# larskaislaniemi/PyLamp

Measured on AMD Instinct MI355X. Metric: stokes_heat_mic_cell_updates_per_s, higher is better.
Workload: dtype f64

## Files before the change

### pylamp_amd/csrc/pl_solver.hip

```cpp
#include "pl_internal.h"
#include <chrono>
#include <cmath>
#include <functional>
#include <limits>

#define TB(tab, k) (tab)[(k) + PL_TOFF]

void pl_launch_heat_rhs(pl_ctx* ctx, const PlHeatOp& op, const double* Told, const double* H, double* rhs);

template <typename T>
struct PlVvOpT {
    PlGeom g;
    const T* etas; const T* etan;
    const T *rdz, *rDz, *rdx, *rDx;
    int slave_x;
    int slave_z0, slave_zL;
    T s0, sL;
    const T* szz; const T* szx;
};
typedef PlVvOpT<double> PlVvOp;
typedef PlVvOpT<float> PlVvOpF;

enum { VV_ZERO = 0, VV_INT = 1, VV_SLAVE = 2 };

// ... 2317 lines not shown
}

template <int NS, int TS>
__global__ __launch_bounds__(mgt_nt(mgt_post_nn(NS, TS))) void k_mg_post(MgTileArgs a) {
    constexpr int H = NS, HC = H + 1, CR = TS + 2 * HC, NN = CR * CR, ECR = TS / 2 + H + 6, ENN = ECR * ECR, NPT = mgt_npt(NN), NT = mgt_nt(NN);
    __shared__ double V[2][2][NN];
    __shared__ double EC[2][ENN];
    __shared__ double TAB[4][CR + 4];
    double* const ES = V[0][0]; double* const EN = V[0][1];
    const PlGeom& g = a.op.g; const PlGeom& gc = a.opc.g;
    const int tid = threadIdx.x;
    const int ty = blockIdx.x / a.tiles_x, tx = blockIdx.x % a.tiles_x;
    const int ti0 = g.gi0 + ty * TS, tj0 = g.gj0 + tx * TS;
    const int ci0 = ti0 - HC, cj0 = tj0 - HC;
    MgtTab t; t.es = ES; t.en = EN; t.rdz = TAB[0]; t.rDz = TAB[1]; t.rdx = TAB[2]; t.rDx = TAB[3];
    mgt_load_table(TAB[0], a.op.rdz, ci0 - 1, CR + 3, g.nz); mgt_load_table(TAB[1], a.op.rDz, ci0 - 1, CR + 3, g.nz);
    mgt_load_table(TAB[2], a.op.rdx, cj0 - 1, CR + 3, g.nx); mgt_load_table(TAB[3], a.op.rDx, cj0 - 1, CR + 3, g.nx);
    const long long P = g.plane;
    const int eI0 = ((ti0 - H) >> 1) - 2, eJ0 = ((tj0 - H) >> 1) - 2;
    MgtC kz[NPT], kx[NPT];
    int depth[NPT];
#pragma unroll
    for (int q = 0; q < NPT; q++) {
        const int idx = tid + q * NT;
        const bool have = idx < NN;
        const int ra = have ? idx / CR : 0, rb = have ? idx % CR : 0, i = ci0 + ra, j = cj0 + rb;
        depth[q] = have ? min(min(ra, CR - 1 - ra), min(rb, CR - 1 - rb)) : -1;
        kz[q] = mgt_classify<true>(a.op, CR, CR, ci0, cj0, ra, rb);
        kx[q] = mgt_classify<false>(a.op, CR, CR, ci0, cj0, ra, rb);
        const bool inmem = i - g.gi0 >= -PL_RING && i - g.gi0 < g.lnz + PL_RING && j - g.gj0 >= -PL_RING && j - g.gj0 < g.lnx + PL_RING;
        const long long c = pl_idx(g, i - g.gi0, j - g.gj0);
        if (kz[q].on) kz[q].f = a.f[c + kz[q].d];
        if (kx[q].on) kx[q].f = a.f[c + (long long)kx[q].d * g.pitch + P];
        if (have) {
            ES[idx] = inmem ? a.op.etas[c] : 0.0; EN[idx] = inmem ? a.op.etan[c] : 0.0;
            V[1][0][idx] = inmem ? a.v[c] : 0.0; V[1][1][idx] = inmem ? a.v[c + P] : 0.0;
        }
    }
    for (int idx = tid; idx < ENN; idx += NT) {
        const int I = eI0 + idx / ECR, J = eJ0 + idx % ECR;
        const bool inmem = I - gc.gi0 >= -PL_RING && I - gc.gi0 < gc.lnz + PL_RING && J - gc.gj0 >= -PL_RING && J - gc.gj0 < gc.lnx + PL_RING;
        const long long cc = pl_idx(gc, I - gc.gi0, J - gc.gj0);
        EC[0][idx] = inmem ? a.ec[cc] : 0.0; EC[1][idx] = inmem ? a.ec[cc + gc.plane] : 0.0;
    }
    __syncthreads();
#pragma unroll
    for (int q = 0; q < NPT; q++) { mgt_coefficients<true>(kz[q], t, CR); mgt_coefficients<false>(kx[q], t, CR); }
    __syncthreads();
    auto ecz = [&](int I, int J) { return EC[0][(I - eI0) * ECR + (J - eJ0)]; };
    auto ecx = [&](int I, int J) { return EC[1][(I - eI0) * ECR + (J - eJ0)]; };
#pragma unroll
    for (int q = 0; q < NPT; q++) {
        const int idx = tid + q * NT;
        if (depth[q] >= HC - H) {
            const int ra = idx / CR, rb = idx % CR, i = ci0 + ra, j = cj0 + rb;
            int d; double s;
            double oz = 0.0, ox = 0.0;
            if (mgt_cls_z(a.op, i, j, d, s) != VV_ZERO) {
                const int jm = j + d;
                const int I0 = i >> 1, I1 = (i + 1) >> 1;
                int Jn = jm >> 1, Jo = (jm & 1) ? Jn + 1 : Jn - 1;
                Jn = min(max(Jn, 0), gc.nx - 2); Jo = min(max(Jo, 0), gc.nx - 2);
                const double pa = 0.5 * (ecz(I0, Jn) + ecz(I1, Jn)), pb = 0.5 * (ecz(I0, Jo) + ecz(I1, Jo));
                oz = s * (V[1][0][idx + d] + (0.75 * pa + 0.25 * pb));
            }
            if (mgt_cls_x(a.op, i, j, d, s) != VV_ZERO) {
                const int im = i + d;
                const int J0 = j >> 1, J1 = (j + 1) >> 1;
                int In = im >> 1, Io = (im & 1) ? In + 1 : In - 1;
                In = min(max(In, 0), gc.nz - 2); Io = min(max(Io, 0), gc.nz - 2);
                const double pa = 0.5 * (ecx(In, J0) + ecx(In, J1)), pb = 0.5 * (ecx(Io, J0) + ecx(Io, J1));
                ox = s * (V[1][1][idx + d * CR] + (0.75 * pa + 0.25 * pb));
            }
            V[0][0][idx] = oz; V[0][1][idx] = ox;
        }
    }
    __syncthreads();
    int cur = 0;
    double pvz[NPT], pvx[NPT];
#pragma unroll
    for (int q = 0; q < NPT; q++) { pvz[q] = 0.0; pvx[q] = 0.0; }
#pragma unroll
    for (int k = 0; k < NS; k++) {
        const int h = H - 1 - k;
#pragma unroll
        for (int q = 0; q < NPT; q++) {
            const int idx = tid + q * NT;
            if (depth[q] >= HC - h) {
                double oz, ox;
                mgt_cheb(kz[q], kx[q], CR, V[cur][0], V[cur][1], pvz[q], pvx[q], k == 0 ? 0.0 : a.c1[k], a.c2[k], oz, ox);
                if (k == NS - 1) {
                    const int ra = idx / CR, rb = idx % CR, i = ci0 + ra, j = cj0 + rb;
                    if (i < g.nz && j < g.nx && i - g.gi0 < g.lnz && j - g.gj0 < g.lnx) {
                        const long long c = pl_idx(g, i - g.gi0, j - g.gj0); a.out[c] = oz * a.oscale; a.out[c + a.out_plane] = ox * a.oscale;
                    }
                } else { V[cur ^ 1][0][idx] = oz; V[cur ^ 1][1][idx] = ox; }
            }
        }
        if (k < NS - 1) { __syncthreads(); cur ^= 1; }
    }
#pragma unroll
    for (int q = 0; q < NPT; q++) {
        const int idx = tid + q * NT;
        if (depth[q] == HC - 1) {
            const int ra = idx / CR, rb = idx % CR, i = ci0 + ra, j = cj0 + rb;
            if (mgt_owns(ra, rb, HC, TS, i, j, g) && i - g.gi0 < g.lnz && j - g.gj0 < g.lnx) {
                const long long c = pl_idx(g, i - g.gi0, j - g.gj0); a.out[c] = 0.0; a.out[c + a.out_plane] = 0.0;
            }
        }
    }
}

#define MGT_TAIL_POOL 18600
struct TailLvl { int base, NR, CR, N; };
#define TL_V(D, buf, c) (pool + (D).base + (2 * (buf) + (c)) * (D).N)
#define TL_F(D, c) (pool + (D).base + (6 + (c)) * (D).N)
#define TL_ES(D) (pool + (D).base + 8 * (D).N)
#define TL_EN(D) (pool + (D).base + 9 * (D).N)
#define TL_TAB(D, k) (pool + (D).base + 10 * (D).N + ((k) < 2 ? (k) * ((D).NR + 3) : 2 * ((D).NR + 3) + ((k) - 2) * ((D).CR + 3)))
#define TL_FOR_NODES(g)                                                                                                     \
    for (int idx = threadIdx.x, nxm_ = (g).nx - 1, pw_ = (nxm_ & (nxm_ - 1)) == 0, sh_ = 31 - __clz(nxm_), i, j;            \
         idx < ((g).nz - 1) * nxm_ && (i = pw_ ? idx >> sh_ : idx / nxm_, j = idx - i * nxm_, true); idx += MGT_NT)
__device__ inline MgtTile mgt_tail_tile(double* pool, const TailLvl& D) {
    MgtTile T; T.ci0 = -1; T.cj0 = -1; T.CR = D.CR; T.NR = D.NR;
    T.t.es = TL_ES(D); T.t.en = TL_EN(D); T.t.rdz = TL_TAB(D, 0); T.t.rDz = TL_TAB(D, 1); T.t.rdx = TL_TAB(D, 2); T.t.rDx = TL_TAB(D, 3);
    return T;
}
__device__ inline void mgt_tail_smooth(double* pool, const TailLevel& L, const TailLvl& D, int& cur, int& prv, int& nxt, int nsweep, double ratio, bool zero_guess) {
    const double lmax = L.lmax, lmin = lmax / ratio;
    const double theta = 0.5 * (lmax + lmin), delta = 0.5 * (lmax - lmin), sigma = theta / delta;
    double rho_old = 1.0 / sigma;
    const MgtTile T = mgt_tail_tile(pool, D);
    for (int k = 0; k < nsweep; k++) {
        double c1, c2;
        if (k == 0) { c1 = 0.0; c2 = 1.0 / theta; }
        else { const double rho = 1.0 / (2.0 * sigma - rho_old); c1 = rho * rho_old; c2 = 2.0 * rho / delta; rho_old = rho; }
        double* const nz_ = TL_V(D, nxt, 0); double* const nx_ = TL_V(D, nxt, 1);
        const double* const cz = TL_V(D, cur, 0); const double* const cx = TL_V(D, cur, 1);
        const bool noprev = k == 1 && zero_guess;
        const double* const pz = noprev ? nullptr : TL_V(D, prv, 0); const double* const px = noprev ? nullptr : TL_V(D, prv, 1);
        TL_FOR_NODES(L.op.g) {
            const int ra = i + 1, rb = j + 1;
            if (k == 0 && zero_guess) T.first(L.op, TL_F(D, 0), TL_F(D, 1), nz_, nx_, c2, ra, rb);
            else {
                double oz, ox;
                T.cheb(L.op, cz, cx, pz, px, TL_F(D, 0), TL_F(D, 1), c1, c2, ra, rb, oz, ox);
                nz_[ra * D.CR + rb] = oz; nx_[ra * D.CR + rb] = ox;
            }
        }
        __syncthreads();
        const int o = prv; prv = cur; cur = nxt; nxt = o;
    }
}
__global__ __launch_bounds__(MGT_NT) void k_mg_tail_lds(TailArgs a) {
    __shared__ double pool[MGT_TAIL_POOL];
    __shared__ TailLvl lv[PL_TAIL_MAX_LEVELS];
    __shared__ int rot[PL_TAIL_MAX_LEVELS];
    const int tid = threadIdx.x;
    for (int k = tid; k < MGT_TAIL_POOL; k += MGT_NT) pool[k] = 0.0;
    if (tid == 0) {
        int q = 0;
        for (int l = 0; l < a.nlev; l++) {
            const PlGeom& g = a.L[l].op.g;
            TailLvl D; D.base = q; D.NR = g.nz + 2; D.CR = g.nx + 2; D.N = D.NR * D.CR;
            q += 10 * D.N + 2 * (D.NR + 3) + 2 * (D.CR + 3);
            lv[l] = D;
        }
    }
    __syncthreads();
    for (int l = 0; l < a.nlev; l++) {
        const TailLevel& L = a.L[l]; const PlGeom& g = L.op.g; const TailLvl D = lv[l];
        for (int idx = tid; idx < g.nz * g.nx; idx += MGT_NT) {
            const int i = idx / g.nx, j = idx - i * g.nx;
            const long long c = pl_idx(g, i - g.gi0, j - g.gj0);
            const int o = (i + 1) * D.CR + (j + 1);
            TL_ES(D)[o] = L.op.etas[c]; TL_EN(D)[o] = L.op.etan[c];
            if (l == 0) { TL_F(D, 0)[o] = L.f[c]; TL_F(D, 1)[o] = L.f[c + g.plane]; }
        }
        mgt_load_table(TL_TAB(D, 0), L.op.rdz, -2, D.NR + 3, g.nz); mgt_load_table(TL_TAB(D, 1), L.op.rDz, -2, D.NR + 3, g.nz);
        mgt_load_table(TL_TAB(D, 2), L.op.rdx, -2, D.CR + 3, g.nx); mgt_load_table(TL_TAB(D, 3), L.op.rDx, -2, D.CR + 3, g.nx);
    }
    __syncthreads();
    for (int l = 0; l < a.nlev; l++) {
        const TailLevel& L = a.L[l]; const PlGeom& g = L.op.g; const TailLvl D = lv[l];
        int cur = 0, prv = 1, nxt = 2;
        if (l == a.nlev - 1) {
            double ratio = 0.4 * g.nz * g.nx; if (ratio < 30.0) ratio = 30.0;
            mgt_tail_smooth(pool, L, D, cur, prv, nxt, a.coarse_sweeps, ratio, true);
            if (tid == 0) rot[l] = cur | (prv << 2) | (nxt << 4);
            break;
        }
        mgt_tail_smooth(pool, L, D, cur, prv, nxt, a.nu_pre, a.ratio, true);
        if (tid == 0) rot[l] = cur | (prv << 2) | (nxt << 4);
        const MgtTile T = mgt_tail_tile(pool, D);
        double* const rz = TL_V(D, nxt, 0); double* const rx = TL_V(D, nxt, 1);
        const double* const cz = TL_V(D, cur, 0); const double* const cx = TL_V(D, cur, 1);
        TL_FOR_NODES(g) {
            const int ra = i + 1, rb = j + 1, o = ra * D.CR + rb;
            int d; double s, Av, dg, vz = 0.0, vx = 0.0;
            if (mgt_cls_z(L.op, i, j, d, s) == VV_INT) { mgt_row_z<true>(T.t, D.CR, cz, cx, o, ra, rb, Av, dg); vz = TL_F(D, 0)[o] - Av; }
            if (mgt_cls_x(L.op, i, j, d, s) == VV_INT) { mgt_row_x<true>(T.t, D.CR, cz, cx, o, ra, rb, Av, dg); vx = TL_F(D, 1)[o] - Av; }
            rz[o] = vz; rx[o] = vx;
        }
        __syncthreads();
        const TailLevel& Cn = a.L[l + 1]; const TailLvl Dc = lv[l + 1];
        double* const fz = TL_F(Dc, 0); double* const fx = TL_F(Dc, 1);
        TL_FOR_NODES(Cn.op.g) {
            const int b0 = (2 * i + 1) * D.CR + (2 * j + 1);
            int d; double s, oz = 0.0, ox = 0.0;
            if (vv_cls_z(Cn.op, i, j, d, s) == VV_INT) {
                const double wz[3] = {0.25, 0.5, 0.25}, wx[4] = {0.125, 0.375, 0.375, 0.125};
#pragma unroll
                for (int u = 0; u < 3; u++)
#pragma unroll
                    for (int w = 0; w < 4; w++) oz += wz[u] * wx[w] * rz[b0 + (u - 1) * D.CR + (w - 1)];
            }
            if (vv_cls_x(Cn.op, i, j, d, s) == VV_INT) {
                const double wz[4] = {0.125, 0.375, 0.375, 0.125}, wx[3] = {0.25, 0.5, 0.25};
#pragma unroll
                for (int u = 0; u < 4; u++)
#pragma unroll
                    for (int w = 0; w < 3; w++) ox += wz[u] * wx[w] * rx[b0 + (u - 1) * D.CR + (w - 1)];
            }
            const int oc = (i + 1) * Dc.CR + (j + 1);
            fz[oc] = oz; fx[oc] = ox;
        }
        __syncthreads();
    }
    __syncthreads();
    for (int l = a.nlev - 2; l >= 0; l--) {
        const TailLevel& L = a.L[l]; const PlGeom& g = L.op.g; const TailLvl D = lv[l];
        const PlGeom& gc = a.L[l + 1].op.g; const TailLvl Dc = lv[l + 1];
        int cur = rot[l] & 3, prv = (rot[l] >> 2) & 3, nxt = (rot[l] >> 4) & 3;
        const int curc = rot[l + 1] & 3;
        const double* const ez = TL_V(Dc, curc, 0); const double* const ex = TL_V(Dc, curc, 1);
        const double* const cz = TL_V(D, cur, 0); const double* const cx = TL_V(D, cur, 1);
        double* const wz_ = TL_V(D, nxt, 0); double* const wx_ = TL_V(D, nxt, 1);
        TL_FOR_NODES(g) {
            const int o = (i + 1) * D.CR + (j + 1);
            int d; double s, oz = 0.0, ox = 0.0;
            if (mgt_cls_z(L.op, i, j, d, s) != VV_ZERO) {
                const int jm = j + d, I0 = i >> 1, I1 = (i + 1) >> 1;
                int Jn = jm >> 1, Jo = (jm & 1) ? Jn + 1 : Jn - 1;
                Jn = min(max(Jn, 0), gc.nx - 2); Jo = min(max(Jo, 0), gc.nx - 2);
                const double pa = 0.5 * (ez[(I0 + 1) * Dc.CR + Jn + 1] + ez[(I1 + 1) * Dc.CR + Jn + 1]);
                const double pb = 0.5 * (ez[(I0 + 1) * Dc.CR + Jo + 1] + ez[(I1 + 1) * Dc.CR + Jo + 1]);
                oz = s * (cz[o + d] + (0.75 * pa + 0.25 * pb));
            }
            if (mgt_cls_x(L.op, i, j, d, s) != VV_ZERO) {
                const int im = i + d, J0 = j >> 1, J1 = (j + 1) >> 1;
                int In = im >> 1, Io = (im & 1) ? In + 1 : In - 1;
                In = min(max(In, 0), gc.nz - 2); Io = min(max(Io, 0), gc.nz - 2);
                const double pa = 0.5 * (ex[(In + 1) * Dc.CR + J0 + 1] + ex[(In + 1) * Dc.CR + J1 + 1]);
                const double pb = 0.5 * (ex[(Io + 1) * Dc.CR + J0 + 1] + ex[(Io + 1) * Dc.CR + J1 + 1]);
                ox = s * (cx[o + d * D.CR] + (0.75 * pa + 0.25 * pb));
            }
            wz_[o] = oz; wx_[o] = ox;
        }
        __syncthreads();
        { const int o = cur; cur = nxt; nxt = o; }
        mgt_tail_smooth(pool, L, D, cur, prv, nxt, a.nu_post, a.ratio, false);
        if (tid == 0) rot[l] = cur | (prv << 2) | (nxt << 4);
        __syncthreads();
    }
    {
        const TailLevel& L = a.L[0]; const PlGeom& g = L.op.g; const TailLvl D = lv[0];
        const int cur = rot[0] & 3;
        const double* const cz = TL_V(D, cur, 0); const double* const cx = TL_V(D, cur, 1);
        for (int idx = tid; idx < g.nz * g.nx; idx += MGT_NT) {
            const int i = idx / g.nx, j = idx - i * g.nx, o = (i + 1) * D.CR + (j + 1);
            const long long c = pl_idx(g, i - g.gi0, j - g.gj0);
            L.v[0][c] = cz[o]; L.v[0][c + g.plane] = cx[o];
        }
    }
}
static bool mg_tail_lds_fits(const PlSolver* S, size_t l) {
    long long need = 0;
    for (size_t q = l; q < S->levels.size(); q++) {
        const PlGeom& g = S->levels[q]->gh.d;
        need += 10LL * (g.nz + 2) * (g.nx + 2) + 2LL * (g.nz + 5) + 2LL * (g.nx + 5);
    }
    return need <= MGT_TAIL_POOL;
}

static void cheb_coeffs(double lmax, double ratio, int n, double* c1, double* c2) {
    const double lmin = lmax / ratio, theta = 0.5 * (lmax + lmin), delta = 0.5 * (lmax - lmin), sigma = theta / delta;
    double rho_old = 1.0 / sigma;
    for (int k = 0; k < n; k++) {
        if (k == 0) { c1[k] = 0.0; c2[k] = 1.0 / theta; }
        else { const double rho = 1.0 / (2.0 * sigma - rho_old); c1[k] = rho * rho_old; c2[k] = 2.0 * rho / delta; rho_old = rho; }
    }
}
static bool mg_fused_level_ok(pl_ctx* ctx, const PlSolver* S, size_t l) {
    if (!S->fused || l + 1 >= S->levels.size() || S->any_line) return false;
    const MgLevel* L = S->levels[l];
    if (L->f32 || L->op.szz) return false;
    const PlGeom& g = L->gh.d;
    int npre_, npost_;
    level_nu(S, l, npre_, npost_);
    if (L->dist) {
        const bool dist_fused = !(getenv("PYLAMP_MG_FUSED_DIST") && atoi(getenv("PYLAMP_MG_FUSED_DIST")) == 0);
        const MgLevel* C = S->levels[l + 1];
        if (!dist_fused || l == 0 || npre_ + 2 > std::min(g.lnz, g.lnx) || npre_ + 3 > PL_RING) return false;
        if (C->dist && std::min(C->gh.d.lnz, C->gh.d.lnx) < 4) return false;
        if ((g.gi0 & 1) || (g.gj0 & 1)) return false;
    } else if (S->levels[l + 1]->dist) return false;
    if ((long long)g.lnz * g.lnx > S->fused_max_nodes) return false;
    if (S->use_tail && l > 0 && (long long)g.nz * g.nx <= S->tail_max_nodes && S->levels.size() - l <= PL_TAIL_MAX_LEVELS) return false;
    int npre, npost;
    level_nu(S, l, npre, npost);
    return npre >= 1 && npre <= 3 && npost >= 1 && npost <= 3;
}
static void vcycle_fused_level(pl_ctx* ctx, PlSolver* S, size_t l, const double* f, double** out, double* final_out, double final_scale,
                               const PlStokesOp* sop, const double* rs, double* z) {
    MgLevel* L = S->levels[l];
    MgLevel* C = S->levels[l + 1];
    const PlGeom& g = L->gh.d;
    int npre, npost;
    level_nu(S, l, npre, npost);
    MgTileArgs a{};
    a.op = L->op; a.opc = C->op;
    a.f = rs ? (const double*)L->f : f; a.fout = L->f; a.v = L->v[0]; a.fc = C->f;
    const int TS = (long long)g.lnz * g.lnx >= S->tile32_min_nodes ? 32 : MGT_TS;
    const int own_z = g.lnz - (g.gi0 + g.lnz == g.nz ? 1 : 0), own_x = g.lnx - (g.gj0 + g.lnx == g.nx ? 1 : 0);
    a.tiles_x = (own_x + TS - 1) / TS;
    const dim3 grid((unsigned)(a.tiles_x * ((own_z + TS - 1) / TS)));
    cheb_coeffs(L->lmax, S->cheb_ratio, npre, a.c1, a.c2);
    if (rs) { a.sop = *sop; a.rs = rs; a.z = z; }
#define MGT_PRE(NS, L0) do { if (TS == 32) hipLaunchKernelGGL((k_mg_pre<NS, L0, 32>), grid, dim3(mgt_nt(mgt_pre_nn(NS, 32))), 0, ctx->stream, a); \
                             else hipLaunchKernelGGL((k_mg_pre<NS, L0, MGT_TS>), grid, dim3(mgt_nt(mgt_pre_nn(NS, MGT_TS))), 0, ctx->stream, a); } while (0)
#define MGT_PRE_X(NS) do { if (TS == 32) hipLaunchKernelGGL((k_mg_pre<NS, false, 32, 1>), grid, dim3(mgt_nt(mgt_pre_nn(NS + 1, 32))), 0, ctx->stream, a); \
                           else hipLaunchKernelGGL((k_mg_pre<NS, false, MGT_TS, 1>), grid, dim3(mgt_nt(mgt_pre_nn(NS + 1, MGT_TS))), 0, ctx->stream, a); } while (0)
    if (L->dist) {
        (void)pl_halo(ctx, g, (double*)a.f, 2, g.plane, npre + 2);
        if (npre == 1) MGT_PRE_X(1); else if (npre == 2) MGT_PRE_X(2); else MGT_PRE_X(3);
        if (!C->dist) (void)pl_gather_blocks(ctx, C->gh.d, C->f, 2, C->gh.d.plane);
    }
    else if (rs) { if (npre == 1) MGT_PRE(1, true); else if (npre == 2) MGT_PRE(2, true); else MGT_PRE(3, true); }
    else { if (npre == 1) MGT_PRE(1, false); else if (npre == 2) MGT_PRE(2, false); else MGT_PRE(3, false); }
#undef MGT_PRE
#undef MGT_PRE_X
    double* ec = nullptr;
    bool wf = false;
    vcycle<double>(ctx, S, l + 1, C->f, &ec, &wf, nullptr, 1.0, 0, nullptr);
    if (L->dist && C->dist) (void)pl_halo(ctx, C->gh.d, ec, 2, C->gh.d.plane, 4);
    a.ec = ec; a.out = final_out ? final_out : L->v[2]; a.oscale = final_out ? final_scale : 1.0; a.out_plane = g.plane;
    cheb_coeffs(L->lmax, S->cheb_ratio, npost, a.c1, a.c2);
#define MGT_POST(NS) do { if (TS == 32) hipLaunchKernelGGL((k_mg_post<NS, 32>), grid, dim3(mgt_nt(mgt_post_nn(NS, 32))), 0, ctx->stream, a); \
                          else hipLaunchKernelGGL((k_mg_post<NS, MGT_TS>), grid, dim3(mgt_nt(mgt_post_nn(NS, MGT_TS))), 0, ctx->stream, a); } while (0)
    if (npost == 1) MGT_POST(1); else if (npost == 2) MGT_POST(2); else MGT_POST(3);
#undef MGT_POST
    *out = final_out ? nullptr : L->v[2];
}

template <typename T>
__global__ __launch_bounds__(256) void k_copy_vel(PlGeom g, const T* __restrict__ e, double* __restrict__ z, double oscale) {
    PL_NODE_PROLOGUE(g)
    (void)i; (void)j;
    z[c] = (double)e[c] * oscale; z[c + g.plane] = (double)e[c + g.plane] * oscale;
}

__global__ __launch_bounds__(256) void k_vv_close_frame(PlVvOp op, double* __restrict__ z) {
    const PlGeom& g = op.g;
    const int t = blockIdx.x * 256 + threadIdx.x;
    int i, j;
    if (t < 3 * g.lnx) { const int q = t / g.lnx; i = q == 0 ? 0 : g.nz - 3 + q; j = g.gj0 + t % g.lnx; }
    else if (t < 3 * g.lnx + 3 * g.lnz) { const int u = t - 3 * g.lnx, q = u / g.lnz; j = q == 0 ? 0 : g.nx - 3 + q; i = g.gi0 + u % g.lnz; }
    else return;
    const int li = i - g.gi0, lj = j - g.gj0;
    if (li < 0 || li >= g.lnz || lj < 0 || lj >= g.lnx) return;
    const long long c = pl_idx(g, li, lj), P = g.plane;
    int moff; double s;
    int cls = vv_cls_z(op, i, j, moff, s);
    if (cls == VV_ZERO) z[c] = 0.0; else if (cls == VV_SLAVE) z[c] = s * z[c + moff];
    cls = vv_cls_x(op, i, j, moff, s);
    if (cls == VV_ZERO) z[c + P] = 0.0; else if (cls == VV_SLAVE) z[c + P] = s * z[c + moff + P];
}

template <typename T>
static int stokes_precond_t(pl_ctx* ctx, PlSolver* S, const double* rs, double* z) {
    PlStokesOp op = ctx->sop;
    MgLevel* L0 = S->levels[0];
    MgLevel* L = L0;
    const PlGeom& g = ctx->sop.g;
    const bool f32 = std::is_same<T, float>::value;
    const double kappa = f32 ? S->kappa : 1.0, fscale = f32 ? S->kappa / S->sigma : 1.0, oscale = f32 ? 1.0 / S->kappa : 1.0;
    int e_last = 0, f_depth = 0;
    const bool deep = level_deep_plan(S, L0, 0, e_last, f_depth);
    ExtViewT<T> V = ext_view<T>(ctx, L0, deep ? f_depth : 0);
    if (L0->dist) {
        if (deep) PL_TRY(pl_halo(ctx, g, (double*)rs, 3, g.plane, f_depth + 1));
        else PL_TRY(pl_halo(ctx, g, (double*)rs + 2 * g.plane, 1, g.plane));
    }
    op.g = V.op.g; op.etas -= V.sh; op.etan -= V.sh; if (op.rho) op.rho -= V.sh;
    op.iKc /= S->schur_scale;
    if constexpr (std::is_same<T, double>::value) {
        if (mg_fused_level_ok(ctx, S, 0)) {
            double* e2 = nullptr;
            vcycle_fused_level(ctx, S, 0, nullptr, &e2, z, 1.0, &op, rs, z);
            PL_HIP(ctx, hipGetLastError());
            S->nprec++;
            return 0;
        }
    }
    int npre0, npost0;
    level_nu(S, 0, npre0, npost0);
    if constexpr (std::is_same<T, double>::value) {
        const double hmean = 0.5 * ((ctx->geom.zc.back() - ctx->geom.zc.front()) / (ctx->nz - 1) + (ctx->geom.xc.back() - ctx->geom.xc.front()) / (ctx->nx - 1));
        const double sig = ctx->sop.Kc / hmean, ik = 1.0 / S->kappa;
        const bool range_ok = std::isfinite(sig) && sig > 0.0 && ik * std::min(1.0, sig) > 1e-30 && ik * std::max(1.0, sig) < 1e22;
        if (S->l0_mixed && S->l0_mixed_now && !S->any_line && range_ok && !L0->dist && !L0->op.szz && g_vv_vec && (g.plane % 2) == 0 && S->levels.size() > 1 && npre0 == 1 && npost0 == 1 &&
            S->fuse_first && ctx->nranks == 1 && !S->levels[1]->dist && !S->levels[1]->f32) {
            MgLevel* C = S->levels[1];
            for (float** q : {&L0->ff, &L0->rf, &L0->vf[0]}) if (!*q) PL_TRY(fmalloc0(ctx, q, (size_t)2 * g.plane * sizeof(float)));
            float* ff = L0->ff; float* rf = L0->rf; float* v1f = L0->vf[0];
            double* vd = L0->v[0];
            PlVvOpT<float> cls{};
// ... 1165 lines not shown
```

Measured before the change: 186.2 million.

## Run coarsest multigrid tail levels on a single wavefront with register-resident stencils

Restructures the LDS multigrid tail kernel so levels small enough to fit in one wavefront (at most 64 nodes) are processed by the first 64 threads only, using wave barriers instead of block-wide __syncthreads. Levels that fit in one block use a per-thread node path whose stencil coefficients and RHS are classified once and kept in registers, rather than recomputed each sweep. Chebyshev coefficients for every level's pre- and post-smoothing sequence are precomputed into a shared table. This targets barrier and recomputation latency in the tiny coarse levels, at the cost of more registers and code complexity, plus reliance on wavefront-synchronous LDS ordering.

Measured after the change: 188.3 million (median of 6 runs). 1.01x the previous value.

```diff
diff --git a/pylamp_amd/csrc/pl_solver.hip b/pylamp_amd/csrc/pl_solver.hip
--- a/pylamp_amd/csrc/pl_solver.hip
+++ b/pylamp_amd/csrc/pl_solver.hip
@@ -2493,8 +2493,171 @@
         const int o = prv; prv = cur; cur = nxt; nxt = o;
     }
 }
+struct TailNode { MgtC kz, kx; int o; bool have; };
+__device__ inline TailNode mgt_tail_enter(double* pool, const TailLevel& L, const TailLvl& D) {
+    TailNode n;
+    const int nxm = L.op.g.nx - 1, idx = threadIdx.x;
+    n.have = idx < (L.op.g.nz - 1) * nxm;
+    const int i = n.have ? idx / nxm : 0, j = n.have ? idx - i * nxm : 0;
+    n.o = (i + 1) * D.CR + (j + 1);
+    n.kz = mgt_classify<true>(L.op, D.CR, D.NR, -1, -1, i + 1, j + 1);
+    n.kx = mgt_classify<false>(L.op, D.CR, D.NR, -1, -1, i + 1, j + 1);
+    if (!n.have) { n.kz.on = n.kz.interior = false; n.kx.on = n.kx.interior = false; }
+    const MgtTile T = mgt_tail_tile(pool, D);
+    mgt_coefficients<true>(n.kz, T.t, D.CR); mgt_coefficients<false>(n.kx, T.t, D.CR);
+    if (n.kz.on) n.kz.f = TL_F(D, 0)[n.kz.cm];
+    if (n.kx.on) n.kx.f = TL_F(D, 1)[n.kx.cm];
+    return n;
+}
+template <bool WAVE> __device__ inline void mgt_tail_sync() {
+    if (WAVE) { asm volatile("s_waitcnt lgkmcnt(0)" ::: "memory"); __builtin_amdgcn_wave_barrier(); }
+    else __syncthreads();
+}
+struct MgtChebSeq {
+    double theta, delta, sigma, rho_old;
+    __device__ inline void init(double lmax, double ratio) {
+        const double lmin = lmax / ratio;
+        theta = 0.5 * (lmax + lmin); delta = 0.5 * (lmax - lmin); sigma = theta / delta; rho_old = 1.0 / sigma;
+    }
+    __device__ inline void next(int k, double& c1, double& c2) {
+        if (k == 0) { c1 = 0.0; c2 = 1.0 / theta; }
+        else { const double rho = 1.0 / (2.0 * sigma - rho_old); c1 = rho * rho_old; c2 = 2.0 * rho / delta; rho_old = rho; }
+    }
+};
+#define MGT_TAIL_CHEB 16
+#define MGT_TAIL_SEQ (2 * PL_TAIL_MAX_LEVELS)
+__device__ inline void mgt_tail_sequence(const TailArgs& a, int s, int& n, double& ratio) {
+    const int l = s % PL_TAIL_MAX_LEVELS;
+    const bool up = s >= PL_TAIL_MAX_LEVELS, coarsest = l == a.nlev - 1;
+    n = 0; ratio = a.ratio;
+    if (l >= a.nlev || (up && coarsest)) return;
+    n = up ? a.nu_post : (coarsest ? a.coarse_sweeps : a.nu_pre);
+    if (coarsest) { const PlGeom& g = a.L[l].op.g; ratio = 0.4 * g.nz * g.nx; if (ratio < 30.0) ratio = 30.0; }
+}
+template <bool WAVE>
+__device__ inline void mgt_tail_smooth_rows(double* pool, const TailLvl& D, const TailNode& n, const double (*ch)[MGT_TAIL_CHEB], double lmax, double ratio,
+                                            int& cur, int& prv, int& nxt, int nsweep, bool zero_guess) {
+    const bool table = nsweep <= MGT_TAIL_CHEB;
+    MgtChebSeq seq; seq.theta = seq.delta = seq.sigma = seq.rho_old = 1.0;
+    if (!table) seq.init(lmax, ratio);
+    double pvz = 0.0, pvx = 0.0;
+    for (int k = 0; k < nsweep; k++) {
+        double c1, c2;
+        if (table) { c1 = ch[0][k]; c2 = ch[1][k]; } else seq.next(k, c1, c2);
+        if (n.have) {
+            double oz, ox;
+            if (k == 0 && zero_guess) {
+                oz = n.kz.on ? (-n.kz.s * c2 * n.kz.f) * n.kz.rdg : 0.0;
+                ox = n.kx.on ? (-n.kx.s * c2 * n.kx.f) * n.kx.rdg : 0.0;
+            } else mgt_cheb(n.kz, n.kx, D.CR, TL_V(D, cur, 0), TL_V(D, cur, 1), pvz, pvx, c1, c2, oz, ox);
+            TL_V(D, nxt, 0)[n.o] = oz; TL_V(D, nxt, 1)[n.o] = ox;
+        }
+        mgt_tail_sync<WAVE>();
+        const int o = prv; prv = cur; cur = nxt; nxt = o;
+    }
+}
+template <bool WAVE>
+__device__ inline void mgt_tail_down(double* pool, const TailArgs& a, const TailLvl* lv, int* rot, const double (*chb)[2][MGT_TAIL_CHEB], int l) {
+    const TailLevel& L = a.L[l]; const PlGeom& g = L.op.g; const TailLvl D = lv[l];
+    const bool coarsest = l == a.nlev - 1, rows = (g.nz - 1) * (g.nx - 1) <= MGT_NT;
+    int cur = 0, prv = 1, nxt = 2, nsweep;
+    double ratio;
+    mgt_tail_sequence(a, l, nsweep, ratio);
+    if (rows) {
+        const TailNode n = mgt_tail_enter(pool, L, D);
+        mgt_tail_smooth_rows<WAVE>(pool, D, n, chb[l], L.lmax, ratio, cur, prv, nxt, nsweep, true);
+        if (threadIdx.x == 0) rot[l] = cur | (prv << 2) | (nxt << 4);
+        if (coarsest) { mgt_tail_sync<WAVE>(); return; }
+        if (n.have) {
+            double v0, vz = 0.0, vx = 0.0;
+            if (n.kz.interior) vz = n.kz.f - mgt_av_z(n.kz, D.CR, TL_V(D, cur, 0), TL_V(D, cur, 1), v0);
+            if (n.kx.interior) vx = n.kx.f - mgt_av_x(n.kx, D.CR, TL_V(D, cur, 0), TL_V(D, cur, 1), v0);
+            TL_V(D, nxt, 0)[n.o] = vz; TL_V(D, nxt, 1)[n.o] = vx;
+        }
+    } else if constexpr (!WAVE) {
+        mgt_tail_smooth(pool, L, D, cur, prv, nxt, nsweep, ratio, true);
+        if (threadIdx.x == 0) rot[l] = cur | (prv << 2) | (nxt << 4);
+        if (coarsest) { mgt_tail_sync<WAVE>(); return; }
+        const MgtTile T = mgt_tail_tile(pool, D);
+        const double* const cz = TL_V(D, cur, 0); const double* const cx = TL_V(D, cur, 1);
+        TL_FOR_NODES(g) {
+            const int ra = i + 1, rb = j + 1, o = ra * D.CR + rb;
+            int d; double s, Av, dg, vz = 0.0, vx = 0.0;
+            if (mgt_cls_z(L.op, i, j, d, s) == VV_INT) { mgt_row_z<true>(T.t, D.CR, cz, cx, o, ra, rb, Av, dg); vz = TL_F(D, 0)[o] - Av; }
+            if (mgt_cls_x(L.op, i, j, d, s) == VV_INT) { mgt_row_x<true>(T.t, D.CR, cz, cx, o, ra, rb, Av, dg); vx = TL_F(D, 1)[o] - Av; }
+            TL_V(D, nxt, 0)[o] = vz; TL_V(D, nxt, 1)[o] = vx;
+        }
+    }
+    mgt_tail_sync<WAVE>();
+    const double* const qz = TL_V(D, nxt, 0); const double* const qx = TL_V(D, nxt, 1);
+    const TailLevel& Cn = a.L[l + 1]; const TailLvl Dc = lv[l + 1];
+    double* const fz = TL_F(Dc, 0); double* const fx = TL_F(Dc, 1);
+    TL_FOR_NODES(Cn.op.g) {
+        const int b0 = (2 * i + 1) * D.CR + (2 * j + 1);
+        int d; double s, oz = 0.0, ox = 0.0;
+        if (vv_cls_z(Cn.op, i, j, d, s) == VV_INT) {
+            const double wz[3] = {0.25, 0.5, 0.25}, wx[4] = {0.125, 0.375, 0.375, 0.125};
+#pragma unroll
+            for (int u = 0; u < 3; u++)
+#pragma unroll
+                for (int w = 0; w < 4; w++) oz += wz[u] * wx[w] * qz[b0 + (u - 1) * D.CR + (w - 1)];
+        }
+        if (vv_cls_x(Cn.op, i, j, d, s) == VV_INT) {
+            const double wz[4] = {0.125, 0.375, 0.375, 0.125}, wx[3] = {0.25, 0.5, 0.25};
+#pragma unroll
+            for (int u = 0; u < 4; u++)
+#pragma unroll
+                for (int w = 0; w < 3; w++) ox += wz[u] * wx[w] * qx[b0 + (u - 1) * D.CR + (w - 1)];
+        }
+        const int oc = (i + 1) * Dc.CR + (j + 1);
+        fz[oc] = oz; fx[oc] = ox;
+    }
+    mgt_tail_sync<WAVE>();
+}
+template <bool WAVE>
+__device__ inline void mgt_tail_up(double* pool, const TailArgs& a, const TailLvl* lv, int* rot, const double (*chb)[2][MGT_TAIL_CHEB], int l) {
+    const TailLevel& L = a.L[l]; const PlGeom& g = L.op.g; const TailLvl D = lv[l];
+    const PlGeom& gc = a.L[l + 1].op.g; const TailLvl Dc = lv[l + 1];
+    int cur = rot[l] & 3, prv = (rot[l] >> 2) & 3, nxt = (rot[l] >> 4) & 3;
+    const int curc = rot[l + 1] & 3;
+    const double* const ez = TL_V(Dc, curc, 0); const double* const ex = TL_V(Dc, curc, 1);
+    const double* const cz = TL_V(D, cur, 0); const double* const cx = TL_V(D, cur, 1);
+    double* const wz_ = TL_V(D, nxt, 0); double* const wx_ = TL_V(D, nxt, 1);
+    TL_FOR_NODES(g) {
+        const int o = (i + 1) * D.CR + (j + 1);
+        int d; double s, oz = 0.0, ox = 0.0;
+        if (mgt_cls_z(L.op, i, j, d, s) != VV_ZERO) {
+            const int jm = j + d, I0 = i >> 1, I1 = (i + 1) >> 1;
+            int Jn = jm >> 1, Jo = (jm & 1) ? Jn + 1 : Jn - 1;
+            Jn = min(max(Jn, 0), gc.nx - 2); Jo = min(max(Jo, 0), gc.nx - 2);
+            const double pa = 0.5 * (ez[(I0 + 1) * Dc.CR + Jn + 1] + ez[(I1 + 1) * Dc.CR + Jn + 1]);
+            const double pb = 0.5 * (ez[(I0 + 1) * Dc.CR + Jo + 1] + ez[(I1 + 1) * Dc.CR + Jo + 1]);
+            oz = s * (cz[o + d] + (0.75 * pa + 0.25 * pb));
+        }
+        if (mgt_cls_x(L.op, i, j, d, s) != VV_ZERO) {
+            const int im = i + d, J0 = j >> 1, J1 = (j + 1) >> 1;
+            int In = im >> 1, Io = (im & 1) ? In + 1 : In - 1;
+            In = min(max(In, 0), gc.nz - 2); Io = min(max(Io, 0), gc.nz - 2);
+            const double pa = 0.5 * (ex[(In + 1) * Dc.CR + J0 + 1] + ex[(In + 1) * Dc.CR + J1 + 1]);
+            const double pb = 0.5 * (ex[(Io + 1) * Dc.CR + J0 + 1] + ex[(Io + 1) * Dc.CR + J1 + 1]);
+            ox = s * (cx[o + d * D.CR] + (0.75 * pa + 0.25 * pb));
+        }
+        wz_[o] = oz; wx_[o] = ox;
+    }
+    mgt_tail_sync<WAVE>();
+    { const int o = cur; cur = nxt; nxt = o; }
+    int nsweep; double ratio;
+    mgt_tail_sequence(a, PL_TAIL_MAX_LEVELS + l, nsweep, ratio);
+    if ((g.nz - 1) * (g.nx - 1) <= MGT_NT) {
+        const TailNode n = mgt_tail_enter(pool, L, D);
+        mgt_tail_smooth_rows<WAVE>(pool, D, n, chb[PL_TAIL_MAX_LEVELS + l], L.lmax, ratio, cur, prv, nxt, nsweep, false);
+    } else if constexpr (!WAVE) mgt_tail_smooth(pool, L, D, cur, prv, nxt, nsweep, ratio, false);
+    if (threadIdx.x == 0) rot[l] = cur | (prv << 2) | (nxt << 4);
+    mgt_tail_sync<WAVE>();
+}
 __global__ __launch_bounds__(MGT_NT) void k_mg_tail_lds(TailArgs a) {
     __shared__ double pool[MGT_TAIL_POOL];
+    __shared__ double chb[MGT_TAIL_SEQ][2][MGT_TAIL_CHEB];
     __shared__ TailLvl lv[PL_TAIL_MAX_LEVELS];
     __shared__ int rot[PL_TAIL_MAX_LEVELS];
     const int tid = threadIdx.x;
@@ -2508,6 +2671,16 @@
             lv[l] = D;
         }
     }
+    if (tid >= 64 && tid < 64 + MGT_TAIL_SEQ) {
+        int n; double ratio;
+        mgt_tail_sequence(a, tid - 64, n, ratio);
+        if (n > 0 && n <= MGT_TAIL_CHEB) {
+            MgtChebSeq seq; seq.init(a.L[(tid - 64) % PL_TAIL_MAX_LEVELS].lmax, ratio);
+            for (int k = 0; k < n; k++) seq.next(k, chb[tid - 64][0][k], chb[tid - 64][1][k]);
+        }
+    }
+    int ls = a.nlev;
+    while (ls > 0 && (a.L[ls - 1].op.g.nz - 1) * (a.L[ls - 1].op.g.nx - 1) <= 64) ls--;
     __syncthreads();
     for (int l = 0; l < a.nlev; l++) {
         const TailLevel& L = a.L[l]; const PlGeom& g = L.op.g; const TailLvl D = lv[l];
@@ -2522,88 +2695,15 @@
         mgt_load_table(TL_TAB(D, 2), L.op.rdx, -2, D.CR + 3, g.nx); mgt_load_table(TL_TAB(D, 3), L.op.rDx, -2, D.CR + 3, g.nx);
     }
     __syncthreads();
-    for (int l = 0; l < a.nlev; l++) {
-        const TailLevel& L = a.L[l]; const PlGeom& g = L.op.g; const TailLvl D = lv[l];
-        int cur = 0, prv = 1, nxt = 2;
-        if (l == a.nlev - 1) {
-            double ratio = 0.4 * g.nz * g.nx; if (ratio < 30.0) ratio = 30.0;
-            mgt_tail_smooth(pool, L, D, cur, prv, nxt, a.coarse_sweeps, ratio, true);
-            if (tid == 0) rot[l] = cur | (prv << 2) | (nxt << 4);
-            break;
-        }
-        mgt_tail_smooth(pool, L, D, cur, prv, nxt, a.nu_pre, a.ratio, true);
-        if (tid == 0) rot[l] = cur | (prv << 2) | (nxt << 4);
-        const MgtTile T = mgt_tail_tile(pool, D);
-        double* const rz = TL_V(D, nxt, 0); double* const rx = TL_V(D, nxt, 1);
-        const double* const cz = TL_V(D, cur, 0); const double* const cx = TL_V(D, cur, 1);
-        TL_FOR_NODES(g) {
-            const int ra = i + 1, rb = j + 1, o = ra * D.CR + rb;
-            int d; double s, Av, dg, vz = 0.0, vx = 0.0;
-            if (mgt_cls_z(L.op, i, j, d, s) == VV_INT) { mgt_row_z<true>(T.t, D.CR, cz, cx, o, ra, rb, Av, dg); vz = TL_F(D, 0)[o] - Av; }
-            if (mgt_cls_x(L.op, i, j, d, s) == VV_INT) { mgt_row_x<true>(T.t, D.CR, cz, cx, o, ra, rb, Av, dg); vx = TL_F(D, 1)[o] - Av; }
-            rz[o] = vz; rx[o] = vx;
+    for (int l = 0; l < ls; l++) mgt_tail_down<false>(pool, a, lv, rot, chb, l);
+    if (ls < a.nlev) {
+        if (tid < 64) {
+            for (int l = ls; l < a.nlev; l++) mgt_tail_down<true>(pool, a, lv, rot, chb, l);
+            for (int l = a.nlev - 2; l >= ls; l--) mgt_tail_up<true>(pool, a, lv, rot, chb, l);
         }
         __syncthreads();
-        const TailLevel& Cn = a.L[l + 1]; const TailLvl Dc = lv[l + 1];
-        double* const fz = TL_F(Dc, 0); double* const fx = TL_F(Dc, 1);
-        TL_FOR_NODES(Cn.op.g) {
-            const int b0 = (2 * i + 1) * D.CR + (2 * j + 1);
-            int d; double s, oz = 0.0, ox = 0.0;
-            if (vv_cls_z(Cn.op, i, j, d, s) == VV_INT) {
-                const double wz[3] = {0.25, 0.5, 0.25}, wx[4] = {0.125, 0.375, 0.375, 0.125};
-#pragma unroll
-                for (int u = 0; u < 3; u++)
-#pragma unroll
-                    for (int w = 0; w < 4; w++) oz += wz[u] * wx[w] * rz[b0 + (u - 1) * D.CR + (w - 1)];
-            }
-            if (vv_cls_x(Cn.op, i, j, d, s) == VV_INT) {
-                const double wz[4] = {0.125, 0.375, 0.375, 0.125}, wx[3] = {0.25, 0.5, 0.25};
-#pragma unroll
-                for (int u = 0; u < 4; u++)
-#pragma unroll
-                    for (int w = 0; w < 3; w++) ox += wz[u] * wx[w] * rx[b0 + (u - 1) * D.CR + (w - 1)];
-            }
-            const int oc = (i + 1) * Dc.CR + (j + 1);
-            fz[oc] = oz; fx[oc] = ox;
-        }
-        __syncthreads();
-    }
-    __syncthreads();
-    for (int l = a.nlev - 2; l >= 0; l--) {
-        const TailLevel& L = a.L[l]; const PlGeom& g = L.op.g; const TailLvl D = lv[l];
-        const PlGeom& gc = a.L[l + 1].op.g; const TailLvl Dc = lv[l + 1];
-        int cur = rot[l] & 3, prv = (rot[l] >> 2) & 3, nxt = (rot[l] >> 4) & 3;
-        const int curc = rot[l + 1] & 3;
-        const double* const ez = TL_V(Dc, curc, 0); const double* const ex = TL_V(Dc, curc, 1);
-        const double* const cz = TL_V(D, cur, 0); const double* const cx = TL_V(D, cur, 1);
-        double* const wz_ = TL_V(D, nxt, 0); double* const wx_ = TL_V(D, nxt, 1);
-        TL_FOR_NODES(g) {
-            const int o = (i + 1) * D.CR + (j + 1);
-            int d; double s, oz = 0.0, ox = 0.0;
-            if (mgt_cls_z(L.op, i, j, d, s) != VV_ZERO) {
-                const int jm = j + d, I0 = i >> 1, I1 = (i + 1) >> 1;
-                int Jn = jm >> 1, Jo = (jm & 1) ? Jn + 1 : Jn - 1;
-                Jn = min(max(Jn, 0), gc.nx - 2); Jo = min(max(Jo, 0), gc.nx - 2);
-                const double pa = 0.5 * (ez[(I0 + 1) * Dc.CR + Jn + 1] + ez[(I1 + 1) * Dc.CR + Jn + 1]);
-                const double pb = 0.5 * (ez[(I0 + 1) * Dc.CR + Jo + 1] + ez[(I1 + 1) * Dc.CR + Jo + 1]);
-                oz = s * (cz[o + d] + (0.75 * pa + 0.25 * pb));
-            }
-            if (mgt_cls_x(L.op, i, j, d, s) != VV_ZERO) {
-                const int im = i + d, J0 = j >> 1, J1 = (j + 1) >> 1;
-                int In = im >> 1, Io = (im & 1) ? In + 1 : In - 1;
-                In = min(max(In, 0), gc.nz - 2); Io = min(max(Io, 0), gc.nz - 2);
-                const double pa = 0.5 * (ex[(In + 1) * Dc.CR + J0 + 1] + ex[(In + 1) * Dc.CR + J1 + 1]);
-                const double pb = 0.5 * (ex[(Io + 1) * Dc.CR + J0 + 1] + ex[(Io + 1) * Dc.CR + J1 + 1]);
-                ox = s * (cx[o + d * D.CR] + (0.75 * pa + 0.25 * pb));
-            }
-            wz_[o] = oz; wx_[o] = ox;
-        }
-        __syncthreads();
-        { const int o = cur; cur = nxt; nxt = o; }
-        mgt_tail_smooth(pool, L, D, cur, prv, nxt, a.nu_post, a.ratio, false);
-        if (tid == 0) rot[l] = cur | (prv << 2) | (nxt << 4);
-        __syncthreads();
-    }
+    }
+    for (int l = min(ls, a.nlev - 1) - 1; l >= 0; l--) mgt_tail_up<false>(pool, a, lv, rot, chb, l);
     {
         const TailLevel& L = a.L[0]; const PlGeom& g = L.op.g; const TailLvl D = lv[0];
         const int cur = rot[0] & 3;
```
